# YAIconvalley/distributed-pipeline

Measured on AMD Instinct MI355X. Metric: train steps/sec (whole node), DiffuSeq-base seq128 DDP at 1/2/4/8 MI355X, higher is better.
Workload: dtype bf16

## Files before the change

### distributed_pipeline_amd/csrc/vocab_sweep.h

```cpp
#pragma once
#include <type_traits>

#include "common.h"
#include "mfma.h"

namespace dpa {

template <int E, int NT>
struct WTile {
  static constexpr int CH = E / 8;
  static constexpr int ROWB = E * 2;
  static constexpr int PER = 64 * CH / NT;
  uint4 r[PER];

  __device__ __forceinline__ void load(const bf16_t* __restrict__ W, int v0, int V, int tid) {
#pragma unroll
    for (int i = 0; i < PER; ++i) {
      const int c = tid + i * NT;
      const int row = c / CH, ch = c % CH;
      const int v = v0 + row;
      if (v < V)
        r[i] = *reinterpret_cast<const uint4*>(W + (int64_t)v * E + ch * 8);
      else
        r[i] = make_uint4(0, 0, 0, 0);
    }
  }
  __device__ __forceinline__ void store(char* lds, int tid) const {
#pragma unroll
    for (int i = 0; i < PER; ++i) {
      const int c = tid + i * NT;
      const int row = c / CH, ch = c % CH;
      *reinterpret_cast<uint4*>(lds + swz<ROWB>(row, ch)) = r[i];
    }
  }
};

template <int E>
__device__ __forceinline__ bf16x8 token_frag(const bf16_t* __restrict__ x, int t, bool tok_ok, int s, int h) {
  bf16x8 f;
  if (tok_ok) f = ld_frag(x + (int64_t)t * E + 16 * s + 8 * h);
  else for (int j = 0; j < 8; ++j) f[j] = 0;
  return f;
}

template <class F>
__device__ __forceinline__ void stage_offsets(float* bt, int v0, int vend, int tid, F offset) {
  if (tid < 64) {
    const int v = v0 + tid;
    bt[tid] = (v < vend) ? offset(v) : -INFINITY;
  }
}

struct SweepBlock {
  int split, tblk, nsplit;
};
__device__ __forceinline__ SweepBlock sweep_block(int xsplit) {
  SweepBlock b;
  b.split = xsplit > 1 ? (int)(blockIdx.x % xsplit) : (int)blockIdx.y;
  b.tblk = xsplit > 1 ? (int)(blockIdx.x / xsplit) : (int)blockIdx.x;
  b.nsplit = xsplit > 1 ? xsplit : (int)gridDim.y;
  return b;
}

inline int pick_splits(int blocks, int chunks, int target_wgs) {
  int s = (target_wgs + blocks - 1) / blocks;
  if (s < 1) s = 1;
  if (s > chunks) s = chunks;
  return s;
}

enum class XcdRound { none, if_split, always };

struct SweepPlan {
  int tb;
  int Sx;
  int vps;
};

inline SweepPlan sweep_plan(int N, int V, int target_wgs, XcdRound xcd) {
  const int tb = (N + 127) / 128, vchunks = (V + 63) / 64;
  int S = pick_splits(tb, vchunks, target_wgs);
  if (vchunks >= 8 && (xcd == XcdRound::always || (xcd == XcdRound::if_split && S > 1))) S = (S + 7) / 8 * 8;
  const int vps = ((vchunks + S - 1) / S) * 64;
  return {tb, (V + vps - 1) / vps, vps};
}

template <class F>
inline void for_head_width(int E, F f) {
  if (E == 128) f(std::integral_constant<int, 128>{});
  else f(std::integral_constant<int, 256>{});
}

}
```

### distributed_pipeline_amd/csrc/xent.hip

```cpp
#include <cstdlib>

#include <type_traits>

#include "common.h"
#include "launchers.h"
#include "mfma.h"
#include "vocab_sweep.h"

namespace dpa {

static constexpr float LN2 = 0.6931471805599453f;

struct BiasOffset {
  const bf16_t* bias;
  __device__ __forceinline__ float operator()(int v) const { return bias ? bf2f(bias[v]) : 0.f; }
};

__device__ __forceinline__ float sel16(const f32x16& a, int i) {
  float v = 0.f;
#pragma unroll
  for (int k = 0; k < 16; ++k) v = (k == i) ? a[k] : v;
  return v;
}

template <int E>
__global__ void __launch_bounds__(256) lxent_fwd_kernel(
    const bf16_t* __restrict__ x, const bf16_t* __restrict__ W, const bf16_t* __restrict__ bias,
    const int64_t* __restrict__ target, int N, int V, int v_per_split, float* __restrict__ loss,
    float* __restrict__ lse_out, float* __restrict__ part_m, float* __restrict__ part_s,
    float* __restrict__ tgt_logit, int xsplit) {
  constexpr int KS = E / 16, ROWB = E * 2;
  __shared__ __attribute__((aligned(16))) char smem[64 * ROWB + 64 * 4];
  char* wt = smem;
  float* bt = reinterpret_cast<float*>(smem + 64 * ROWB);

  const auto [split, tblk, nsplit] = sweep_block(xsplit);
  const int tid = threadIdx.x, lane = tid & 63, w = tid >> 6, h = lane >> 5;
  const int t = tblk * 128 + w * 32 + (lane & 31);
  const bool tok_ok = t < N;
  bf16x8 xf[KS];
#pragma unroll
  for (int s = 0; s < KS; ++s) xf[s] = token_frag<E>(x, t, tok_ok, s, h);
  const int64_t tg = tok_ok ? target[t] : -1;

  const int vbeg = split * v_per_split;
  const int vend = min(V, vbeg + v_per_split);
  if (!__syncthreads_or(tg >= 0 && tg < V)) {
    if (h == 0 && tok_ok) {
      if (nsplit == 1) {
        loss[t] = 0.f;
        lse_out[t] = 0.f;
      } else {
        part_m[(int64_t)split * N + t] = 0.f;
        part_s[(int64_t)split * N + t] = 1.f;
      }
    }
    return;
  }
  float m = -1e30f, ssum = 0.f, tl = -INFINITY;

  WTile<E, 256> stage;
  if (vbeg < vend) stage.load(W, vbeg, V, tid);
  for (int v0 = vbeg; v0 < vend; v0 += 64) {
    stage.store(wt, tid);
    stage_offsets(bt, v0, vend, tid, BiasOffset{bias});
    __syncthreads();
    if (v0 + 64 < vend) stage.load(W, v0 + 64, V, tid);

    f32x16 acc[2];
#pragma unroll
    for (int vt = 0; vt < 2; ++vt) {
#pragma unroll
      for (int g = 0; g < 4; ++g) {
        const f32x4 bv = *reinterpret_cast<const f32x4*>(bt + vt * 32 + 8 * g + 4 * h);
#pragma unroll
        for (int r = 0; r < 4; ++r) acc[vt][4 * g + r] = bv[r];
      }
#pragma unroll
      for (int s = 0; s < KS; ++s)
        acc[vt] = mfma32(lds_frag<ROWB>(wt, vt * 32 + (lane & 31), 2 * s + h), xf[s], acc[vt]);
    }
    float tmax = -INFINITY;
#pragma unroll
    for (int vt = 0; vt < 2; ++vt)
#pragma unroll
      for (int i = 0; i < 16; i += 2) tmax = fmaxf(tmax, fmaxf(acc[vt][i], acc[vt][i + 1]));
    const float mn = fmaxf(m, tmax * LOG2E);
    float add = 0.f;
#pragma unroll
    for (int vt = 0; vt < 2; ++vt)
#pragma unroll
      for (int i = 0; i < 16; ++i) add += fexp2(fmaf(acc[vt][i], LOG2E, -mn));
    ssum = ssum * fexp2(m - mn) + add;
    m = mn;
    const int64_t r = tg - v0;
    if (r >= 0 && r < 64 && v0 + r < vend) {
      const int rr = (int)r & 31, vt = (int)r >> 5;
      if (((rr >> 2) & 1) == h) {
        const int i = (rr & 3) + 4 * (rr >> 3);
        tl = vt ? sel16(acc[1], i) : sel16(acc[0], i);
      }
    }
    __syncthreads();
  }
  const float m2 = __shfl_xor(m, 32, 64), s2 = __shfl_xor(ssum, 32, 64);
  const float tl2 = __shfl_xor(tl, 32, 64);
  const float M = fmaxf(m, m2);
  const float S = ssum * fexp2(m - M) + s2 * fexp2(m2 - M);
  tl = fmaxf(tl, tl2);
  if (h == 0 && tok_ok) {
    if (nsplit == 1) {
      const bool valid = tg >= 0 && tg < V;
      const float lse = (M + log2f(S)) * LN2;
      loss[t] = valid ? lse - tl : 0.f;
      lse_out[t] = lse;
    } else {
      part_m[(int64_t)split * N + t] = M;
      part_s[(int64_t)split * N + t] = S;
      if (tl > -INFINITY) tgt_logit[t] = tl;
    }
  }
}

__global__ void __launch_bounds__(256) lxent_combine_kernel(
    const float* __restrict__ part_m, const float* __restrict__ part_s,
    const float* __restrict__ tgt_logit, const int64_t* __restrict__ target, int N, int V, int S,
    float* __restrict__ loss, float* __restrict__ lse_out) {
  const int t = blockIdx.x * blockDim.x + threadIdx.x;
  if (t >= N) return;
  float M = -1e30f;
  for (int s = 0; s < S; ++s) M = fmaxf(M, part_m[(int64_t)s * N + t]);
  float sum = 0.f;
  for (int s = 0; s < S; ++s) sum += part_s[(int64_t)s * N + t] * fexp2(part_m[(int64_t)s * N + t] - M);
  const float lse = (M + log2f(sum)) * LN2;
  const int64_t tg = target[t];
  const bool valid = tg >= 0 && tg < V;
  loss[t] = valid ? lse - tgt_logit[t] : 0.f;
  lse_out[t] = lse;
}

template <int E>
__global__ void __launch_bounds__(256) lxent_dx_kernel(
    const bf16_t* __restrict__ x, const bf16_t* __restrict__ W, const bf16_t* __restrict__ bias,
    const int64_t* __restrict__ target, const float* __restrict__ lse, const float* __restrict__ dloss,
    int N, int V, int v_per_split, bf16_t* __restrict__ dx, float* __restrict__ dx_acc) {
  constexpr int KS = E / 16, ROWB = E * 2, KT = E / 32;
  __shared__ __attribute__((aligned(16))) char smem[64 * ROWB + 64 * 4];
  char* wt = smem;
  float* bt = reinterpret_cast<float*>(smem + 64 * ROWB);

  const int tid = threadIdx.x, lane = tid & 63, w = tid >> 6, h = lane >> 5;
  const int t = blockIdx.x * 128 + w * 32 + (lane & 31);
  const bool tok_ok = t < N;
  bf16x8 xf[KS];
#pragma unroll
  for (int s = 0; s < KS; ++s) xf[s] = token_frag<E>(x, t, tok_ok, s, h);
  const int64_t tg = tok_ok ? target[t] : -1;
  const bool valid = tok_ok && tg >= 0 && tg < V;
  const float g = valid ? dloss[t] : 0.f;
  const float lse2 = tok_ok ? lse[t] * LOG2E : 0.f;

  const int vbeg = blockIdx.y * v_per_split;
  const int vend = min(V, vbeg + v_per_split);
  f32x16 dacc[KT];
#pragma unroll
  for (int k = 0; k < KT; ++k) dacc[k] = zero16();

  WTile<E, 256> stage;
  if (vbeg < vend) stage.load(W, vbeg, V, tid);
  for (int v0 = vbeg; v0 < vend; v0 += 64) {
    stage.store(wt, tid);
    stage_offsets(bt, v0, vend, tid, BiasOffset{bias});
    __syncthreads();
    if (v0 + 64 < vend) stage.load(W, v0 + 64, V, tid);

#pragma unroll
    for (int vt = 0; vt < 2; ++vt) {
      f32x16 acc;
#pragma unroll
      for (int g4 = 0; g4 < 4; ++g4) {
        const f32x4 bv = *reinterpret_cast<const f32x4*>(bt + vt * 32 + 8 * g4 + 4 * h);
#pragma unroll
        for (int r = 0; r < 4; ++r) acc[4 * g4 + r] = bv[r];
      }
#pragma unroll
      for (int s = 0; s < KS; ++s)
        acc = mfma32(lds_frag<ROWB>(wt, vt * 32 + (lane & 31), 2 * s + h), xf[s], acc);
#pragma unroll
      for (int i = 0; i < 16; ++i) acc[i] = g * fexp2(fmaf(acc[i], LOG2E, -lse2));
      const int64_t rt = tg - (v0 + vt * 32);
      if (rt >= 0 && rt < 32 && tg < vend && ((rt >> 2) & 1) == h) {
        const int it = ((int)rt & 3) + 4 * ((int)rt >> 3);
#pragma unroll
        for (int i = 0; i < 16; ++i) acc[i] -= (i == it) ? g : 0.f;
      }
#pragma unroll
      for (int s = 0; s < 2; ++s) {
        const bf16x8 af = acc_to_frag(acc, s);
#pragma unroll
        for (int kt = 0; kt < KT; ++kt)
          dacc[kt] = mfma32(af, lds_tr_frag<ROWB>(wt, vt * 32 + 16 * s, kt * 32, lane), dacc[kt]);
      }
    }
    __syncthreads();
  }
  const int tb = blockIdx.x * 128 + w * 32;
#pragma unroll
  for (int kt = 0; kt < KT; ++kt) {
#pragma unroll
    for (int i = 0; i < 16; ++i) {
      const int tt = tb + acc_row(i, h);
      if (tt < N) {
        const int64_t o = (int64_t)tt * E + kt * 32 + (lane & 31);
        if (dx_acc) atomicAdd(dx_acc + o, dacc[kt][i]);
        else dx[o] = f2bf(dacc[kt][i]);
      }
    }
  }
}

template <int E>
__global__ void __launch_bounds__(256, E == 128 ? 2 : 1) lxent_fwd_dx_kernel(
    const bf16_t* __restrict__ x, const bf16_t* __restrict__ W, const bf16_t* __restrict__ bias,
    const int64_t* __restrict__ target, int N, int V, float* __restrict__ loss,
    float* __restrict__ lse_out, float* __restrict__ dxu, int vps, float* __restrict__ part) {
  constexpr int KS = E / 16, ROWB = E * 2, KT = E / 32;
  __shared__ __attribute__((aligned(16))) char smem[64 * ROWB + 64 * 4];
  const int v_lo = part ? (int)blockIdx.y * vps : 0;
  const int v_hi = part ? min(V, v_lo + vps) : V;
  char* wt = smem;
  float* bt = reinterpret_cast<float*>(smem + 64 * ROWB);

  const int tid = threadIdx.x, lane = tid & 63, w = tid >> 6, h = lane >> 5;
  const int t = blockIdx.x * 128 + w * 32 + (lane & 31);
  const bool tok_ok = t < N;
  bf16x8 xf[KS];
#pragma unroll
  for (int s = 0; s < KS; ++s) xf[s] = token_frag<E>(x, t, tok_ok, s, h);
  const int64_t tg = tok_ok ? target[t] : -1;
  f32x16 dacc[KT];
#pragma unroll
  for (int k = 0; k < KT; ++k) dacc[k] = zero16();
  float m = -1e30f, l = 0.f, tl = -INFINITY;

  WTile<E, 256> stage;
  stage.load(W, v_lo, V, tid);
  for (int v0 = v_lo; v0 < v_hi; v0 += 64) {
    stage.store(wt, tid);
    stage_offsets(bt, v0, v_hi, tid, BiasOffset{bias});
    __syncthreads();
    if (v0 + 64 < v_hi) stage.load(W, v0 + 64, V, tid);

#pragma unroll
    for (int vt = 0; vt < 2; ++vt) {
      f32x16 acc;
#pragma unroll
      for (int g = 0; g < 4; ++g) {
        const f32x4 bv = *reinterpret_cast<const f32x4*>(bt + vt * 32 + 8 * g + 4 * h);
#pragma unroll
        for (int r = 0; r < 4; ++r) acc[4 * g + r] = bv[r];
      }
#pragma unroll
      for (int s = 0; s < KS; ++s)
        acc = mfma32(lds_frag<ROWB>(wt, vt * 32 + (lane & 31), 2 * s + h), xf[s], acc);
      const int64_t r = tg - (v0 + vt * 32);
      if (r >= 0 && r < 32 && ((((int)r >> 2) & 1) == h)) tl = sel16(acc, ((int)r & 3) + 4 * ((int)r >> 3));
      float tmax = -INFINITY;
#pragma unroll
      for (int i = 0; i < 16; ++i) tmax = fmaxf(tmax, acc[i]);
      tmax = fmaxf(tmax, __shfl_xor(tmax, 32, 64)) * LOG2E;
      if (__any(tmax > m + 8.f)) {
        const float mn = fmaxf(m, tmax);
        const float alpha = fexp2(m - mn);
        m = mn;
        l *= alpha;
#pragma unroll
        for (int i = 0; i < 16; ++i) {
          const float f = __shfl(alpha, acc_row(i, h), 64);
#pragma unroll
          for (int kt = 0; kt < KT; ++kt) dacc[kt][i] *= f;
        }
      }
#pragma unroll
      for (int i = 0; i < 16; ++i) {
        const float pr = fexp2(fmaf(acc[i], LOG2E, -m));
        l += pr;
        acc[i] = pr;
      }
#pragma unroll
      for (int s = 0; s < 2; ++s) {
        const bf16x8 af = acc_to_frag(acc, s);
#pragma unroll
        for (int kt = 0; kt < KT; ++kt)
          dacc[kt] = mfma32(af, lds_tr_frag<ROWB>(wt, vt * 32 + 16 * s, kt * 32, lane), dacc[kt]);
      }
    }
    __syncthreads();
  }
  l += __shfl_xor(l, 32, 64);
  tl = fmaxf(tl, __shfl_xor(tl, 32, 64));
  if (part) {
    const int S = gridDim.y, sp = blockIdx.y;
    float* pm = part;
    float* pl = pm + (int64_t)S * N;
    float* pt = pl + (int64_t)S * N;
    float* pu = pt + (int64_t)S * N;
    if (h == 0 && tok_ok) {
      pm[(int64_t)sp * N + t] = m;
      pl[(int64_t)sp * N + t] = l;
      pt[(int64_t)sp * N + t] = tl;
    }
    const int tb0 = blockIdx.x * 128 + w * 32;
#pragma unroll
    for (int i = 0; i < 16; ++i) {
      const int tt = tb0 + acc_row(i, h);
      if (tt < N) {
#pragma unroll
        for (int kt = 0; kt < KT; ++kt) pu[((int64_t)sp * N + tt) * E + kt * 32 + (lane & 31)] = dacc[kt][i];
      }
    }
    return;
  }
  const bool valid = tok_ok && tg >= 0 && tg < V;
  const float lse = (m + log2f(l)) * LN2;
  if (h == 0 && tok_ok) {
    loss[t] = valid ? lse - tl : 0.f;
    lse_out[t] = lse;
  }
  const float inv_l = valid ? 1.f / l : 0.f;
  const int tb = blockIdx.x * 128 + w * 32;
#pragma unroll
  for (int i = 0; i < 16; ++i) {
    const int src = acc_row(i, h);
    const float f = __shfl(inv_l, src, 64);
    const int64_t tgi = __shfl(tg, src, 64);
    const int tt = tb + src;
    if (tt < N) {
#pragma unroll
      for (int kt = 0; kt < KT; ++kt) {
        const int k = kt * 32 + (lane & 31);
        float vv = 0.f;
        if (f != 0.f) vv = dacc[kt][i] * f - bf2f(W[tgi * E + k]);
        dxu[(int64_t)tt * E + k] = vv;
      }
    }
  }
}

template <int E>
__global__ void __launch_bounds__(256) lxent_fwd_dx_combine_kernel(
    const float* __restrict__ part, int S, const bf16_t* __restrict__ W, const int64_t* __restrict__ target,
    int N, int V, float* __restrict__ loss, float* __restrict__ lse_out, float* __restrict__ dxu) {
  const int64_t idx = (int64_t)blockIdx.x * blockDim.x + threadIdx.x;
  if (idx >= (int64_t)N * E) return;
  const int t = (int)(idx / E), k = (int)(idx % E);
  const float* pm = part;
  const float* pl = pm + (int64_t)S * N;
  const float* pt = pl + (int64_t)S * N;
  const float* pu = pt + (int64_t)S * N;
  float M = -1e30f, tl = -INFINITY;
  for (int s = 0; s < S; ++s) {
    M = fmaxf(M, pm[(int64_t)s * N + t]);
    tl = fmaxf(tl, pt[(int64_t)s * N + t]);
  }
  float L = 0.f, u = 0.f;
  for (int s = 0; s < S; ++s) {
    const float f = fexp2(pm[(int64_t)s * N + t] - M);
    L += pl[(int64_t)s * N + t] * f;
    u += pu[((int64_t)s * N + t) * E + k] * f;
  }
  const int64_t tg = target[t];
  const bool valid = tg >= 0 && tg < V;
  const float lse = (M + log2f(L)) * LN2;
  if (k == 0) {
    loss[t] = valid ? lse - tl : 0.f;
    lse_out[t] = lse;
  }
  dxu[(int64_t)t * E + k] = valid ? u / L - bf2f(W[tg * E + k]) : 0.f;
}

template <int E, bool ONEHOT = true>
__global__ void __launch_bounds__(512) lxent_dw_kernel(
    const bf16_t* __restrict__ x, const bf16_t* __restrict__ W, const bf16_t* __restrict__ bias,
    const int64_t* __restrict__ target, const float* __restrict__ lse, const float* __restrict__ dloss,
    int N, int V, int t_per_split, float* __restrict__ dW, float* __restrict__ db, float* __restrict__ ws) {
  constexpr int KS = E / 16, ROWB = E * 2, KT = E / 32, CH = E / 8;
  __shared__ __attribute__((aligned(16))) char smem[64 * ROWB + 3 * 64 * 4];
  char* xt = smem;
  float* s_lse = reinterpret_cast<float*>(smem + 64 * ROWB);
  float* s_g = s_lse + 64;
  int* s_tg = reinterpret_cast<int*>(s_g + 64);

  const int tid = threadIdx.x, lane = tid & 63, w = tid >> 6, h = lane >> 5;
  if (w < 4) __builtin_amdgcn_s_setprio(1);
  const int vw = blockIdx.x * 256 + w * 32;
  const int v = vw + (lane & 31);
  const bool v_ok = v < V;
  bf16x8 wf[KS];
#pragma unroll
  for (int s = 0; s < KS; ++s) {
    if (v_ok) wf[s] = ld_frag(W + (int64_t)v * E + 16 * s + 8 * h);
    else for (int j = 0; j < 8; ++j) wf[s][j] = 0;
  }
  const float bv = v_ok ? (bias ? bf2f(bias[v]) : 0.f) : -INFINITY;

  f32x16 dacc[KT];
#pragma unroll
  for (int k = 0; k < KT; ++k) dacc[k] = zero16();
  float dbs = 0.f;

  const int tbeg = blockIdx.y * t_per_split;
  const int tend = min(N, tbeg + t_per_split);
  constexpr int PER = 64 * CH / 512;
  uint4 xr[PER];
  float r_lse = 0.f, r_g = 0.f;
  int r_tg = -1;
  auto load_tile = [&](int t0) {
#pragma unroll
    for (int i = 0; i < PER; ++i) {
      const int c = tid + i * 512;
      const int t = t0 + c / CH;
      xr[i] = t < tend ? *reinterpret_cast<const uint4*>(x + (int64_t)t * E + (c % CH) * 8)
                       : make_uint4(0, 0, 0, 0);
    }
    if (tid < 64) {
      const int t = t0 + tid;
      const bool ok = t < tend;
      const int64_t tg = ok ? target[t] : -1;
      const bool valid = ok && tg >= 0 && tg < V;
      r_lse = ok ? lse[t] * LOG2E : 0.f;
      r_g = valid ? dloss[t] : 0.f;
      r_tg = valid ? (int)tg : -1;
    }
  };
  if (tbeg < tend) load_tile(tbeg);
  for (int t0 = tbeg; t0 < tend; t0 += 64) {
#pragma unroll
    for (int i = 0; i < PER; ++i) {
      const int c = tid + i * 512;
      *reinterpret_cast<uint4*>(xt + swz<ROWB, true>(c / CH, c % CH)) = xr[i];
    }
    if (tid < 64) {
      s_lse[tid] = r_lse;
      s_g[tid] = r_g;
      s_tg[tid] = r_tg;
    }
    __syncthreads();
    if (t0 + 64 < tend) load_tile(t0 + 64);
#pragma unroll
    for (int tt = 0; tt < 2; ++tt) {
      f32x16 acc;
#pragma unroll
      for (int i = 0; i < 16; ++i) acc[i] = bv;
#pragma unroll
      for (int s = 0; s < KS; ++s)
        acc = mfma32(lds_frag<ROWB, true>(xt, tt * 32 + (lane & 31), 2 * s + h), wf[s], acc);
      auto softmax_grad = [&](auto oh) {
        constexpr bool OH = decltype(oh)::value;
#pragma unroll
        for (int g4 = 0; g4 < 4; ++g4) {
          const int rb = tt * 32 + 8 * g4 + 4 * h;
          const f32x4 l4 = *reinterpret_cast<const f32x4*>(s_lse + rb);
          const f32x4 g4v = *reinterpret_cast<const f32x4*>(s_g + rb);
          int tgs[4] = {-1, -1, -1, -1};
          if constexpr (OH) {
            const int4 t4 = *reinterpret_cast<const int4*>(s_tg + rb);
            tgs[0] = t4.x; tgs[1] = t4.y; tgs[2] = t4.z; tgs[3] = t4.w;
          }
#pragma unroll
          for (int r = 0; r < 4; ++r) {
            const int i = 4 * g4 + r;
            const float gp = g4v[r] * fexp2(fmaf(acc[i], LOG2E, -l4[r]));
            const float d = (OH && tgs[r] == v) ? gp - g4v[r] : gp;
            acc[i] = d;
            dbs += d;
          }
        }
      };
      bool hit = false;
      if constexpr (ONEHOT) {
        const int tgl = s_tg[tt * 32 + (lane & 31)];
        hit = __any(tgl >= vw && tgl < vw + 32);
      }
      if (hit) softmax_grad(std::true_type{});
      else softmax_grad(std::false_type{});
#pragma unroll
      for (int s = 0; s < 2; ++s) {
        const bf16x8 af = acc_to_frag(acc, s);
#pragma unroll
        for (int kt = 0; kt < KT; ++kt)
          dacc[kt] = mfma32(af, lds_tr_frag<ROWB, true>(xt, tt * 32 + 16 * s, kt * 32, lane), dacc[kt]);
      }
    }
    __syncthreads();
  }
  dbs += __shfl_xor(dbs, 32, 64);
  float* const pw = ws ? ws + (int64_t)blockIdx.y * V * (E + 1) : nullptr;
  if (h == 0 && v_ok && db) {
    if (pw) pw[(int64_t)V * E + v] = dbs;
    else db[v] += dbs;
  }
#pragma unroll
  for (int kt = 0; kt < KT; ++kt) {
#pragma unroll
    for (int i = 0; i < 16; ++i) {
      const int vv = vw + acc_row(i, h);
      if (vv < V) {
        const int64_t o = (int64_t)vv * E + kt * 32 + (lane & 31);
        if (pw) pw[o] = dacc[kt][i];
        else dW[o] += dacc[kt][i];
      }
    }
  }
}

__global__ void __launch_bounds__(256) xent_split_reduce_kernel(const float* __restrict__ ws, int64_t stride,
                                                                int splits, int64_t n, float* __restrict__ dst) {
  const int64_t i = (int64_t)blockIdx.x * blockDim.x + threadIdx.x;
  if (i >= n) return;
  float a = dst[i];
  for (int sp = 0; sp < splits; ++sp) a += ws[(int64_t)sp * stride + i];
  dst[i] = a;
}

__global__ void __launch_bounds__(256) f32_to_bf16_kernel(const float* __restrict__ a,
                                                         bf16_t* __restrict__ b, int64_t n) {
  const int64_t i = ((int64_t)blockIdx.x * blockDim.x + threadIdx.x) * 4;
  if (i + 3 < n) {
    f32x4 v = *reinterpret_cast<const f32x4*>(a + i);
    uint2 p;
    p.x = pack_bf2(v[0], v[1]);
    p.y = pack_bf2(v[2], v[3]);
    *reinterpret_cast<uint2*>(b + i) = p;
  } else {
    for (int64_t k = i; k < n; ++k) b[k] = f2bf(a[k]);
  }
}

static SweepPlan fwd_plan(int N, int V) { return sweep_plan(N, V, 1024, XcdRound::always); }

int64_t lxent_workspace_floats(int N, int V) { return (2 * (int64_t)fwd_plan(N, V).Sx + 1) * N + 64; }

void launch_lxent_fwd(const uint16_t* x, const uint16_t* W, const uint16_t* b, const int64_t* tgt,
                      int N, int V, int E, float* loss, float* lse, float* ws, hipStream_t s) {
  const SweepPlan p = fwd_plan(N, V);
  float* pm = ws;
  float* ps = ws + (int64_t)p.Sx * N;
  float* tl = ws + 2 * (int64_t)p.Sx * N;
  const bool per_xcd = p.Sx == 8;
  const dim3 grid = per_xcd ? dim3(p.tb * 8) : dim3(p.tb, p.Sx);
  for_head_width(E, [&](auto e) {
    hipLaunchKernelGGL(lxent_fwd_kernel<e()>, grid, dim3(256), 0, s, x, W, b, tgt, N, V, p.vps, loss, lse, pm,
                       ps, tl, per_xcd ? 8 : 0);
  });
  if (p.Sx > 1)
    hipLaunchKernelGGL(lxent_combine_kernel, dim3((N + 255) / 256), dim3(256), 0, s, pm, ps, tl,
                       tgt, N, V, p.Sx, loss, lse);
}

static SweepPlan fwd_dx_plan(int N, int V) { return sweep_plan(N, V, 768, XcdRound::none); }

int64_t lxent_fwd_dx_workspace_floats(int N, int V, int E) {
  const int S = fwd_dx_plan(N, V).Sx;
  return S > 1 ? (int64_t)S * N * (3 + E) : 0;
}

void launch_lxent_fwd_dx(const uint16_t* x, const uint16_t* W, const uint16_t* b, const int64_t* tgt,
                         int N, int V, int E, float* loss, float* lse, float* dxu, hipStream_t s, float* ws) {
  const SweepPlan p = fwd_dx_plan(N, V);
  for_head_width(E, [&](auto e) {
    if (p.Sx > 1 && ws != nullptr) {
      hipLaunchKernelGGL(lxent_fwd_dx_kernel<e()>, dim3(p.tb, p.Sx), dim3(256), 0, s, x, W, b, tgt, N, V, loss,
                         lse, dxu, p.vps, ws);
      const int64_t n = (int64_t)N * E;
      hipLaunchKernelGGL(lxent_fwd_dx_combine_kernel<e()>, dim3((unsigned)((n + 255) / 256)), dim3(256), 0, s, ws,
                         p.Sx, W, tgt, N, V, loss, lse, dxu);
    } else {
      hipLaunchKernelGGL(lxent_fwd_dx_kernel<e()>, dim3(p.tb), dim3(256), 0, s, x, W, b, tgt, N, V, loss, lse,
                         dxu, V, nullptr);
    }
  });
}

bool lxent_dx_needs_acc(int N) { return (N + 127) / 128 < 512; }

void launch_lxent_dx(const uint16_t* x, const uint16_t* W, const uint16_t* b, const int64_t* tgt,
                     const float* lse, const float* dloss, int N, int V, int E, uint16_t* dx,
                     float* dx_acc, hipStream_t s) {
  const SweepPlan p = sweep_plan(N, V, dx_acc ? 1024 : 0, XcdRound::none);
  for_head_width(E, [&](auto e) {
    hipLaunchKernelGGL(lxent_dx_kernel<e()>, dim3(p.tb, p.Sx), dim3(256), 0, s, x, W, b, tgt, lse, dloss, N, V,
                       p.vps, dx, p.Sx > 1 ? dx_acc : nullptr);
  });
  if (p.Sx > 1) {
    const int64_t n = (int64_t)N * E;
    hipLaunchKernelGGL(f32_to_bf16_kernel, dim3((unsigned)((n / 4 + 255) / 256 + 1)), dim3(256), 0,
                       s, dx_acc, dx, n);
  }
}

static void lxent_dw_plan(int N, int V, int& vb, int& tps, int& TSx) {
  vb = (V + 255) / 256;
  const int tchunks = (N + 63) / 64;
  const int TS = pick_splits(vb, tchunks, 960);
  tps = ((tchunks + TS - 1) / TS) * 64;
  TSx = (N + tps - 1) / tps;
}

int64_t lxent_dw_ws_floats(int N, int V, int E) {
  int vb, tps, TSx;
  lxent_dw_plan(N, V, vb, tps, TSx);
  return TSx > 1 ? (int64_t)TSx * V * (E + 1) : 0;
}

void launch_lxent_dw(const uint16_t* x, const uint16_t* W, const uint16_t* b, const int64_t* tgt,
                     const float* lse, const float* dloss, int N, int V, int E, float* dW, float* db,
                     hipStream_t s, bool onehot, float* ws) {
  int vb, tps, TSx;
  lxent_dw_plan(N, V, vb, tps, TSx);
  float* wsp = TSx > 1 ? ws : nullptr;
#define DPA_LXDW(EE, OH)                                                                                \
  hipLaunchKernelGGL((lxent_dw_kernel<EE, OH>), dim3(vb, TSx), dim3(512), 0, s, (const bf16_t*)x,        \
                     (const bf16_t*)W, (const bf16_t*)b, tgt, lse, dloss, N, V, tps, dW, db, wsp)
  if (E == 128) {
    if (onehot) DPA_LXDW(128, true); else DPA_LXDW(128, false);
  } else {
    if (onehot) DPA_LXDW(256, true); else DPA_LXDW(256, false);
  }
#undef DPA_LXDW
  if (wsp) {
    const int64_t stride = (int64_t)V * (E + 1), nw = (int64_t)V * E;
    hipLaunchKernelGGL(xent_split_reduce_kernel, dim3((unsigned)((nw + 255) / 256)), dim3(256), 0, s,
                       (const float*)wsp, stride, TSx, nw, dW);
    if (db)
      hipLaunchKernelGGL(xent_split_reduce_kernel, dim3((unsigned)((V + 255) / 256)), dim3(256), 0, s,
                         (const float*)(wsp + nw), stride, TSx, (int64_t)V, db);
  }
}

}
```

Before: 6.195.

## Stream vocab/token tiles through a 3-stage LDS ring with direct buffer-to-LDS loads

New measurement: 6.245 (median of 6 runs). About the same (+0.8%).

```diff
diff --git a/distributed_pipeline_amd/csrc/vocab_sweep.h b/distributed_pipeline_amd/csrc/vocab_sweep.h
--- a/distributed_pipeline_amd/csrc/vocab_sweep.h
+++ b/distributed_pipeline_amd/csrc/vocab_sweep.h
@@ -1,5 +1,6 @@
 #pragma once
 #include <type_traits>
+#include <utility>
 
 #include "common.h"
 #include "mfma.h"
@@ -35,6 +36,205 @@
   }
 };
 
+typedef __attribute__((address_space(3))) void lds_void;
+
+struct RingSched {
+  int R;
+  constexpr int slot(int tile) const { return ((tile % R) + R) % R; }
+  constexpr int tiles_in_flight_at_wait() const { return R - 2; }
+  constexpr int published(int tile) const { return tile; }
+  constexpr int first_read(int tile) const { return tile; }
+  constexpr int last_read(int tile) const { return tile + 1; }
+  constexpr int fill_after(int tile) const { return tile <= R - 2 ? -0x7fffffff : tile - R + 1; }
+  constexpr int barriers(int T) const { return T > 0 ? T : 0; }
+};
+constexpr bool ring_schedule_ok(RingSched s, int T) {
+  if (s.R < 3 || s.tiles_in_flight_at_wait() != 1) return false;
+  if (s.barriers(T) != T) return false;
+  for (int j = 0; j < T + s.R - 1; ++j) {
+    if (j < T && s.first_read(j) < s.published(j)) return false;
+    if (j < T && s.published(j) < s.fill_after(j)) return false;
+    if (j >= s.R && s.slot(j) != s.slot(j - s.R)) return false;
+    if (j >= s.R && s.fill_after(j) < s.last_read(j - s.R)) return false;
+  }
+  return true;
+}
+constexpr bool ring_schedule_ok_all(RingSched s) {
+  const int trips[8] = {0, 1, 2, s.R - 1, s.R, s.R + 1, s.R + 2, 477};
+  for (int k = 0; k < 8; ++k)
+    if (!ring_schedule_ok(s, trips[k])) return false;
+  return true;
+}
+
+template <int N>
+__device__ __forceinline__ void ring_wait_vm() { asm volatile("s_waitcnt vmcnt(%0)" ::"i"(N) : "memory"); }
+__device__ __forceinline__ void ring_barrier() { asm volatile("s_waitcnt lgkmcnt(0)\n\ts_barrier" ::: "memory"); }
+
+template <int OFF>
+__device__ __forceinline__ bf16x8 ring_rd128(uint32_t a) {
+  bf16x8 f;
+  asm volatile("ds_read_b128 %0, %1 offset:%2" : "=v"(f) : "v"(a), "i"(OFF));
+  return f;
+}
+template <int OFF>
+__device__ __forceinline__ f32x4 ring_rd_f4(uint32_t a) {
+  f32x4 f;
+  asm volatile("ds_read_b128 %0, %1 offset:%2" : "=v"(f) : "v"(a), "i"(OFF));
+  return f;
+}
+typedef __attribute__((ext_vector_type(4))) int i32x4;
+template <int OFF>
+__device__ __forceinline__ i32x4 ring_rd_i4(uint32_t a) {
+  i32x4 f;
+  asm volatile("ds_read_b128 %0, %1 offset:%2" : "=v"(f) : "v"(a), "i"(OFF));
+  return f;
+}
+template <int OFF>
+__device__ __forceinline__ int ring_rd_i1(uint32_t a) {
+  int f;
+  asm volatile("ds_read_b32 %0, %1 offset:%2" : "=v"(f) : "v"(a), "i"(OFF));
+  return f;
+}
+template <int OFF>
+__device__ __forceinline__ bf16x4 ring_rdtr(uint32_t a) {
+  bf16x4 f;
+  asm volatile("ds_read_b64_tr_b16 %0, %1 offset:%2" : "=v"(f) : "v"(a), "i"(OFF));
+  return f;
+}
+__device__ __forceinline__ void ring_wr_b32(uint32_t a, uint32_t v) {
+  asm volatile("ds_write_b32 %0, %1" ::"v"(a), "v"(v) : "memory");
+}
+template <int N, class T>
+__device__ __forceinline__ void ring_lgkm(T& f) { asm volatile("s_waitcnt lgkmcnt(%1)" : "+v"(f) : "i"(N)); }
+template <int N, class T>
+__device__ __forceinline__ void ring_lgkm(T& f, T& g) {
+  asm volatile("s_waitcnt lgkmcnt(%2)" : "+v"(f), "+v"(g) : "i"(N));
+}
+
+__device__ __forceinline__ uint32_t ring_ld_u16(const void* p) {
+  uint32_t v;
+  asm volatile("global_load_ushort %0, %1, off" : "=v"(v) : "v"(p));
+  return v;
+}
+__device__ __forceinline__ uint32_t ring_ld_b32(const void* p) {
+  uint32_t v;
+  asm volatile("global_load_dword %0, %1, off" : "=v"(v) : "v"(p));
+  return v;
+}
+__device__ __forceinline__ int64_t ring_ld_b64(const void* p) {
+  int64_t v;
+  asm volatile("global_load_dwordx2 %0, %1, off" : "=v"(v) : "v"(p));
+  return v;
+}
+template <int N, class T>
+__device__ __forceinline__ void ring_wait_vm_on(T& a) {
+  asm volatile("s_waitcnt vmcnt(%1)" : "+v"(a) : "i"(N) : "memory");
+}
+
+template <int E, int NW, int R, int SIDE, bool LEG>
+struct TileRing {
+  static constexpr int ROWB = E * 2, CH = E / 8, TILE = 64 * ROWB;
+  static constexpr int PER = TILE / 1024 / NW;
+  static constexpr int TAIL = SIDE * 256;
+  static constexpr int BYTES = R * (TILE + TAIL);
+  static constexpr int KS = E / 16, KT = E / 32;
+  static_assert(ROWB % 256 == 0 && ROWB <= 1024 && PER >= 1 && PER * NW * 1024 == TILE, "tile shape");
+
+  char* smem;
+  uint32_t base;
+  uint32_t off[PER];
+  uint32_t rdA[KS];
+  uint32_t rdT[KT][2];
+  int wv;
+
+  __device__ __forceinline__ void init(char* smem_, int tid) {
+    smem = smem_;
+    base = (uint32_t)reinterpret_cast<uintptr_t>((const __attribute__((address_space(3))) char*)smem_);
+    const int lane = tid & 63, h = lane >> 5;
+    wv = __builtin_amdgcn_readfirstlane(tid >> 6);
+#pragma unroll
+    for (int j = 0; j < PER; ++j) {
+      const int row = (wv * PER + j) * (64 / CH) + lane / CH, phys = lane % CH;
+      off[j] = (uint32_t)(row * ROWB + ((phys ^ swz_x256<LEG>(row)) << 4));
+    }
+#pragma unroll
+    for (int s = 0; s < KS; ++s) rdA[s] = (uint32_t)swz<ROWB, LEG>(lane & 31, 2 * s + h);
+    const int g = lane >> 4, li = lane & 15, q = li >> 2, p = li & 3;
+#pragma unroll
+    for (int kt = 0; kt < KT; ++kt) {
+      const int col = kt * 32 + 16 * (g & 1) + 4 * p, ra = 4 * h + q;
+      rdT[kt][0] = (uint32_t)(swz<ROWB, LEG>(ra, col >> 3) + (col & 7) * 2);
+      rdT[kt][1] = (uint32_t)(swz<ROWB, LEG>(ra + 8, col >> 3) + (col & 7) * 2);
+    }
+  }
+  __device__ __forceinline__ uint32_t tile_addr(int slot) const { return base + (uint32_t)(slot * TILE); }
+  __device__ __forceinline__ uint32_t tail_addr(int slot) const { return base + (uint32_t)(R * TILE + slot * TAIL); }
+
+  __device__ __forceinline__ void fill(int slot, const bf16_t* __restrict__ src, int row0, int rows) const {
+    const int n = __builtin_amdgcn_readfirstlane(min(max(rows - row0, 0), 64));
+    const bf16_t* p = src + (n > 0 ? (int64_t)row0 * E : 0);
+    const auto rs = __builtin_amdgcn_make_buffer_rsrc(const_cast<bf16_t*>(p), (short)0, n * ROWB, 0x00020000);
+#pragma unroll
+    for (int j = 0; j < PER; ++j)
+      __builtin_amdgcn_raw_ptr_buffer_load_lds(rs, (lds_void*)(smem + slot * TILE + (wv * PER + j) * 1024), 16,
+                                               off[j], 0, 0, 0);
+  }
+};
+
+template <class Ring, int VT, int J>
+__device__ __forceinline__ void ring_logits_step(f32x16& acc, bf16x8 (&f)[4], const Ring& r, uint32_t ta,
+                                                 const bf16x8 (&b)[Ring::KS]) {
+  constexpr int KS = Ring::KS, N = KS - 1 - J < 3 ? KS - 1 - J : 3;
+  ring_lgkm<N>(f[J % 4]);
+  acc = mfma32(f[J % 4], b[J], acc);
+  if constexpr (J + 4 < KS) f[J % 4] = ring_rd128<VT * 32 * Ring::ROWB>(ta + r.rdA[J + 4]);
+}
+template <class Ring, int VT, int... J>
+__device__ __forceinline__ void ring_logits_steps(f32x16& acc, bf16x8 (&f)[4], const Ring& r, uint32_t ta,
+                                                  const bf16x8 (&b)[Ring::KS], std::integer_sequence<int, J...>) {
+  (ring_logits_step<Ring, VT, J>(acc, f, r, ta, b), ...);
+}
+template <class Ring, int VT, class Init>
+__device__ __forceinline__ void ring_logits(f32x16& acc, const Ring& r, uint32_t ta,
+                                            const bf16x8 (&b)[Ring::KS], Init init) {
+  bf16x8 f[4];
+#pragma unroll
+  for (int j = 0; j < 4; ++j) f[j] = ring_rd128<VT * 32 * Ring::ROWB>(ta + r.rdA[j]);
+  init(acc);
+  ring_logits_steps<Ring, VT>(acc, f, r, ta, b, std::make_integer_sequence<int, Ring::KS>{});
+}
+
+struct TrChunk {
+  bf16x4 a[4], b[4];
+};
+template <class Ring, int VT, int C>
+__device__ __forceinline__ void ring_tr_issue(TrChunk& c, const Ring& r, uint32_t ta) {
+  constexpr int S = C / (Ring::KT / 4), KT0 = 4 * (C % (Ring::KT / 4)), OFF = (VT * 32 + 16 * S) * Ring::ROWB;
+#pragma unroll
+  for (int k = 0; k < 4; ++k) {
+    c.a[k] = ring_rdtr<OFF>(ta + r.rdT[KT0 + k][0]);
+    c.b[k] = ring_rdtr<OFF>(ta + r.rdT[KT0 + k][1]);
+  }
+}
+template <class Ring, int VT, int C = 0>
+__device__ __forceinline__ void ring_acc_mfma(f32x16 (&dacc)[Ring::KT], const f32x16& acc, const Ring& r,
+                                              uint32_t ta, TrChunk& cur) {
+  constexpr int NCH = Ring::KT / 2, S = C / (Ring::KT / 4), KT0 = 4 * (C % (Ring::KT / 4));
+  constexpr int P = C + 1 < NCH ? 8 : 0;
+  const bf16x8 af = acc_to_frag(acc, S);
+  TrChunk nxt;
+  ring_lgkm<6>(cur.a[0], cur.b[0]);
+  if constexpr (C + 1 < NCH) ring_tr_issue<Ring, VT, C + 1>(nxt, r, ta);
+  dacc[KT0] = mfma32(af, cat44(cur.a[0], cur.b[0]), dacc[KT0]);
+  ring_lgkm<P + 4>(cur.a[1], cur.b[1]);
+  dacc[KT0 + 1] = mfma32(af, cat44(cur.a[1], cur.b[1]), dacc[KT0 + 1]);
+  ring_lgkm<P + 2>(cur.a[2], cur.b[2]);
+  dacc[KT0 + 2] = mfma32(af, cat44(cur.a[2], cur.b[2]), dacc[KT0 + 2]);
+  ring_lgkm<P>(cur.a[3], cur.b[3]);
+  dacc[KT0 + 3] = mfma32(af, cat44(cur.a[3], cur.b[3]), dacc[KT0 + 3]);
+  if constexpr (C + 1 < NCH) ring_acc_mfma<Ring, VT, C + 1>(dacc, acc, r, ta, nxt);
+}
+
 template <int E>
 __device__ __forceinline__ bf16x8 token_frag(const bf16_t* __restrict__ x, int t, bool tok_ok, int s, int h) {
   bf16x8 f;
diff --git a/distributed_pipeline_amd/csrc/xent.hip b/distributed_pipeline_amd/csrc/xent.hip
--- a/distributed_pipeline_amd/csrc/xent.hip
+++ b/distributed_pipeline_amd/csrc/xent.hip
@@ -15,6 +15,14 @@
   const bf16_t* bias;
   __device__ __forceinline__ float operator()(int v) const { return bias ? bf2f(bias[v]) : 0.f; }
 };
+
+constexpr int FWD_DX_STAGES = 3, DW_STAGES = 3;
+template <int E> using FwdDxRing = TileRing<E, 4, FWD_DX_STAGES, 1, false>;
+template <int E> using DwRing = TileRing<E, 8, DW_STAGES, 3, true>;
+static_assert(ring_schedule_ok_all(RingSched{FWD_DX_STAGES}), "lxent_fwd_dx ring schedule");
+static_assert(ring_schedule_ok_all(RingSched{DW_STAGES}), "lxent_dw ring schedule");
+static_assert(2 * FwdDxRing<128>::BYTES <= 160 * 1024 && FwdDxRing<256>::BYTES <= 160 * 1024 &&
+              DwRing<256>::BYTES <= 160 * 1024, "the rings of a CU's resident blocks fit its LDS");
 
 __device__ __forceinline__ float sel16(const f32x16& a, int i) {
   float v = 0.f;
@@ -224,14 +232,16 @@
     const bf16_t* __restrict__ x, const bf16_t* __restrict__ W, const bf16_t* __restrict__ bias,
     const int64_t* __restrict__ target, int N, int V, float* __restrict__ loss,
     float* __restrict__ lse_out, float* __restrict__ dxu, int vps, float* __restrict__ part) {
-  constexpr int KS = E / 16, ROWB = E * 2, KT = E / 32;
-  __shared__ __attribute__((aligned(16))) char smem[64 * ROWB + 64 * 4];
+  constexpr int KS = E / 16, KT = E / 32;
+  using Ring = FwdDxRing<E>;
+  constexpr int R = FWD_DX_STAGES, PER = Ring::PER;
+  __shared__ __attribute__((aligned(1024))) char smem[Ring::BYTES];
   const int v_lo = part ? (int)blockIdx.y * vps : 0;
   const int v_hi = part ? min(V, v_lo + vps) : V;
-  char* wt = smem;
-  float* bt = reinterpret_cast<float*>(smem + 64 * ROWB);
 
   const int tid = threadIdx.x, lane = tid & 63, w = tid >> 6, h = lane >> 5;
+  Ring ring;
+  ring.init(smem, tid);
   const int t = blockIdx.x * 128 + w * 32 + (lane & 31);
   const bool tok_ok = t < N;
   bf16x8 xf[KS];
@@ -243,26 +253,64 @@
   for (int k = 0; k < KT; ++k) dacc[k] = zero16();
   float m = -1e30f, l = 0.f, tl = -INFINITY;
 
-  WTile<E, 256> stage;
-  stage.load(W, v_lo, V, tid);
-  for (int v0 = v_lo; v0 < v_hi; v0 += 64) {
-    stage.store(wt, tid);
-    stage_offsets(bt, v0, v_hi, tid, BiasOffset{bias});
-    __syncthreads();
-    if (v0 + 64 < v_hi) stage.load(W, v0 + 64, V, tid);
-
-#pragma unroll
-    for (int vt = 0; vt < 2; ++vt) {
+  const bool side_wave = ring.wv == 0;
+  auto side_load = [&](int j) -> uint32_t {
+    return bias ? ring_ld_u16(bias + min(v_lo + 64 * j + tid, v_hi - 1)) : 0u;
+  };
+  auto side_store = [&](int j, int slot, uint32_t raw) {
+    const float o = v_lo + 64 * j + tid < v_hi ? (bias ? bf2f((bf16_t)raw) : 0.f) : -INFINITY;
+    ring_wr_b32(ring.tail_addr(slot) + 4 * tid, __float_as_uint(o));
+  };
+  uint32_t snext = 0;
+  {
+    uint32_t sraw[R];
+    if (side_wave) {
+#pragma unroll
+      for (int j = 0; j < R; ++j) sraw[j] = side_load(j);
+    }
+#pragma unroll
+    for (int j = 0; j < R - 1; ++j) ring.fill(j, W, v_lo + 64 * j, v_hi);
+    if (side_wave) {
+#pragma unroll
+      for (int j = 0; j < R; ++j) ring_wait_vm_on<(R - 1) * PER>(sraw[j]);
+#pragma unroll
+      for (int j = 0; j < R - 1; ++j) side_store(j, j, sraw[j]);
+      snext = sraw[R - 1];
+    }
+  }
+  const int tiles = (v_hi - v_lo + 63) / 64;
+  int slot = 0;
+  for (int it = 0; it < tiles; ++it) {
+    const int v0 = v_lo + 64 * it;
+    ring_wait_vm_on<PER>(snext);
+    ring_barrier();
+    {
+      const int fslot = slot == 0 ? R - 1 : slot - 1;
+      if (side_wave) {
+        side_store(it + R - 1, fslot, snext);
+        snext = side_load(it + R);
+      }
+      ring.fill(fslot, W, v0 + 64 * (R - 1), v_hi);
+    }
+    const uint32_t ta = ring.tile_addr(slot), sa = ring.tail_addr(slot) + 16 * h;
+    slot = slot == R - 1 ? 0 : slot + 1;
+
+    auto subtile = [&](auto vtc) {
+      constexpr int vt = decltype(vtc)::value;
       f32x16 acc;
-#pragma unroll
-      for (int g = 0; g < 4; ++g) {
-        const f32x4 bv = *reinterpret_cast<const f32x4*>(bt + vt * 32 + 8 * g + 4 * h);
-#pragma unroll
-        for (int r = 0; r < 4; ++r) acc[4 * g + r] = bv[r];
-      }
-#pragma unroll
-      for (int s = 0; s < KS; ++s)
-        acc = mfma32(lds_frag<ROWB>(wt, vt * 32 + (lane & 31), 2 * s + h), xf[s], acc);
+      f32x4 bv[4];
+#pragma unroll
+      for (int g = 0; g < 4; ++g) bv[g] = ring_rd_f4<vt * 128>(sa + 32 * g);
+      ring_logits<Ring, vt>(acc, ring, ta, xf, [&](f32x16& a) {
+        ring_lgkm<4>(bv[0], bv[1]);
+        ring_lgkm<4>(bv[2], bv[3]);
+#pragma unroll
+        for (int g = 0; g < 4; ++g)
+#pragma unroll
+          for (int r = 0; r < 4; ++r) a[4 * g + r] = bv[g][r];
+      });
+      TrChunk tr;
+      ring_tr_issue<Ring, vt, 0>(tr, ring, ta);
       const int64_t r = tg - (v0 + vt * 32);
       if (r >= 0 && r < 32 && ((((int)r >> 2) & 1) == h)) tl = sel16(acc, ((int)r & 3) + 4 * ((int)r >> 3));
       float tmax = -INFINITY;
@@ -287,16 +335,12 @@
         l += pr;
         acc[i] = pr;
       }
-#pragma unroll
-      for (int s = 0; s < 2; ++s) {
-        const bf16x8 af = acc_to_frag(acc, s);
-#pragma unroll
-        for (int kt = 0; kt < KT; ++kt)
-          dacc[kt] = mfma32(af, lds_tr_frag<ROWB>(wt, vt * 32 + 16 * s, kt * 32, lane), dacc[kt]);
-      }
-    }
-    __syncthreads();
-  }
+      ring_acc_mfma<Ring, vt>(dacc, acc, ring, ta, tr);
+    };
+    subtile(std::integral_constant<int, 0>{});
+    subtile(std::integral_constant<int, 1>{});
+  }
+  ring_wait_vm<0>();
   l += __shfl_xor(l, 32, 64);
   tl = fmaxf(tl, __shfl_xor(tl, 32, 64));
   if (part) {
@@ -384,15 +428,14 @@
     const bf16_t* __restrict__ x, const bf16_t* __restrict__ W, const bf16_t* __restrict__ bias,
     const int64_t* __restrict__ target, const float* __restrict__ lse, const float* __restrict__ dloss,
     int N, int V, int t_per_split, float* __restrict__ dW, float* __restrict__ db, float* __restrict__ ws) {
-  constexpr int KS = E / 16, ROWB = E * 2, KT = E / 32, CH = E / 8;
-  __shared__ __attribute__((aligned(16))) char smem[64 * ROWB + 3 * 64 * 4];
-  char* xt = smem;
-  float* s_lse = reinterpret_cast<float*>(smem + 64 * ROWB);
-  float* s_g = s_lse + 64;
-  int* s_tg = reinterpret_cast<int*>(s_g + 64);
+  constexpr int KS = E / 16, KT = E / 32;
+  using Ring = DwRing<E>;
+  constexpr int R = DW_STAGES, PER = Ring::PER;
+  __shared__ __attribute__((aligned(1024))) char smem[Ring::BYTES];
 
   const int tid = threadIdx.x, lane = tid & 63, w = tid >> 6, h = lane >> 5;
-  if (w < 4) __builtin_amdgcn_s_setprio(1);
+  Ring ring;
+  ring.init(smem, tid);
   const int vw = blockIdx.x * 256 + w * 32;
   const int v = vw + (lane & 31);
   const bool v_ok = v < V;
@@ -411,67 +454,98 @@
 
   const int tbeg = blockIdx.y * t_per_split;
   const int tend = min(N, tbeg + t_per_split);
-  constexpr int PER = 64 * CH / 512;
-  uint4 xr[PER];
-  float r_lse = 0.f, r_g = 0.f;
-  int r_tg = -1;
-  auto load_tile = [&](int t0) {
-#pragma unroll
-    for (int i = 0; i < PER; ++i) {
-      const int c = tid + i * 512;
-      const int t = t0 + c / CH;
-      xr[i] = t < tend ? *reinterpret_cast<const uint4*>(x + (int64_t)t * E + (c % CH) * 8)
-                       : make_uint4(0, 0, 0, 0);
-    }
-    if (tid < 64) {
-      const int t = t0 + tid;
-      const bool ok = t < tend;
-      const int64_t tg = ok ? target[t] : -1;
-      const bool valid = ok && tg >= 0 && tg < V;
-      r_lse = ok ? lse[t] * LOG2E : 0.f;
-      r_g = valid ? dloss[t] : 0.f;
-      r_tg = valid ? (int)tg : -1;
-    }
+  const int tiles = (tend - tbeg + 63) / 64;
+  const bool side_wave = ring.wv == 0;
+  struct Side {
+    uint32_t l, g;
+    int64_t t;
   };
-  if (tbeg < tend) load_tile(tbeg);
-  for (int t0 = tbeg; t0 < tend; t0 += 64) {
-#pragma unroll
-    for (int i = 0; i < PER; ++i) {
-      const int c = tid + i * 512;
-      *reinterpret_cast<uint4*>(xt + swz<ROWB, true>(c / CH, c % CH)) = xr[i];
-    }
-    if (tid < 64) {
-      s_lse[tid] = r_lse;
-      s_g[tid] = r_g;
-      s_tg[tid] = r_tg;
-    }
-    __syncthreads();
-    if (t0 + 64 < tend) load_tile(t0 + 64);
-#pragma unroll
-    for (int tt = 0; tt < 2; ++tt) {
+  auto side_load = [&](int j) {
+    const int t = max(min(tbeg + 64 * j + tid, tend - 1), 0);
+    return Side{ring_ld_b32(lse + t), ring_ld_b32(dloss + t), ring_ld_b64(target + t)};
+  };
+  auto side_store = [&](int j, int slot, const Side& sd) {
+    const bool ok = tbeg + 64 * j + tid < tend;
+    const bool valid = ok && sd.t >= 0 && sd.t < V;
+    const uint32_t a = ring.tail_addr(slot) + 4 * tid;
+    ring_wr_b32(a, __float_as_uint(ok ? __uint_as_float(sd.l) * LOG2E : 0.f));
+    ring_wr_b32(a + 256, valid ? sd.g : 0u);
+    ring_wr_b32(a + 512, (uint32_t)(valid ? (int)sd.t : -1));
+  };
+  Side snext{0u, 0u, 0};
+  if (tiles > 0) {
+    Side sraw[R];
+    if (side_wave) {
+#pragma unroll
+      for (int j = 0; j < R; ++j) sraw[j] = side_load(j);
+    }
+#pragma unroll
+    for (int j = 0; j < R - 1; ++j) ring.fill(j, x, tbeg + 64 * j, tend);
+    if (side_wave) {
+#pragma unroll
+      for (int j = 0; j < R; ++j) {
+        ring_wait_vm_on<(R - 1) * PER>(sraw[j].l);
+        ring_wait_vm_on<(R - 1) * PER>(sraw[j].g);
+        ring_wait_vm_on<(R - 1) * PER>(sraw[j].t);
+      }
+#pragma unroll
+      for (int j = 0; j < R - 1; ++j) side_store(j, j, sraw[j]);
+      snext = sraw[R - 1];
+    }
+  }
+  int slot = 0;
+  for (int it = 0; it < tiles; ++it) {
+    ring_wait_vm_on<PER>(snext.l);
+    ring_wait_vm_on<PER>(snext.g);
+    ring_wait_vm_on<PER>(snext.t);
+    const uint32_t ta = ring.tile_addr(slot), sa = ring.tail_addr(slot);
+    ring_barrier();
+    {
+      const int fslot = slot == 0 ? R - 1 : slot - 1;
+      if (side_wave) {
+        side_store(it + R - 1, fslot, snext);
+        snext = side_load(it + R);
+      }
+      ring.fill(fslot, x, tbeg + 64 * (it + R - 1), tend);
+    }
+    slot = slot == R - 1 ? 0 : slot + 1;
+    auto set_bias = [&](f32x16& a) {
+#pragma unroll
+      for (int i = 0; i < 16; ++i) a[i] = bv;
+    };
+    auto subtile = [&](auto ttc) {
+      constexpr int tt = decltype(ttc)::value;
       f32x16 acc;
-#pragma unroll
-      for (int i = 0; i < 16; ++i) acc[i] = bv;
-#pragma unroll
-      for (int s = 0; s < KS; ++s)
-        acc = mfma32(lds_frag<ROWB, true>(xt, tt * 32 + (lane & 31), 2 * s + h), wf[s], acc);
+      ring_logits<Ring, tt>(acc, ring, ta, wf, set_bias);
+      int tgl = 0;
+      if constexpr (ONEHOT) tgl = ring_rd_i1<512 + tt * 128>(sa + 4 * (lane & 31));
+      f32x4 l4[4], g4v[4];
+#pragma unroll
+      for (int g4 = 0; g4 < 4; ++g4) {
+        l4[g4] = ring_rd_f4<tt * 128>(sa + 32 * g4 + 16 * h);
+        g4v[g4] = ring_rd_f4<256 + tt * 128>(sa + 32 * g4 + 16 * h);
+      }
+      TrChunk tr;
       auto softmax_grad = [&](auto oh) {
         constexpr bool OH = decltype(oh)::value;
 #pragma unroll
         for (int g4 = 0; g4 < 4; ++g4) {
-          const int rb = tt * 32 + 8 * g4 + 4 * h;
-          const f32x4 l4 = *reinterpret_cast<const f32x4*>(s_lse + rb);
-          const f32x4 g4v = *reinterpret_cast<const f32x4*>(s_g + rb);
+          if (g4 == 0) ring_lgkm<6>(l4[0], g4v[0]);
+          else if (g4 == 1) ring_lgkm<12>(l4[1], g4v[1]);
+          else if (g4 == 2) ring_lgkm<10>(l4[2], g4v[2]);
+          else ring_lgkm<8>(l4[3], g4v[3]);
+          if (g4 == 0) ring_tr_issue<Ring, tt, 0>(tr, ring, ta);
           int tgs[4] = {-1, -1, -1, -1};
           if constexpr (OH) {
-            const int4 t4 = *reinterpret_cast<const int4*>(s_tg + rb);
-            tgs[0] = t4.x; tgs[1] = t4.y; tgs[2] = t4.z; tgs[3] = t4.w;
+            i32x4 t4 = ring_rd_i4<512 + tt * 128>(sa + 32 * g4 + 16 * h);
+            ring_lgkm<0>(t4);
+            tgs[0] = t4[0]; tgs[1] = t4[1]; tgs[2] = t4[2]; tgs[3] = t4[3];
           }
 #pragma unroll
           for (int r = 0; r < 4; ++r) {
             const int i = 4 * g4 + r;
-            const float gp = g4v[r] * fexp2(fmaf(acc[i], LOG2E, -l4[r]));
-            const float d = (OH && tgs[r] == v) ? gp - g4v[r] : gp;
+            const float gp = g4v[g4][r] * fexp2(fmaf(acc[i], LOG2E, -l4[g4][r]));
+            const float d = (OH && tgs[r] == v) ? gp - g4v[g4][r] : gp;
             acc[i] = d;
             dbs += d;
           }
@@ -479,21 +553,17 @@
       };
       bool hit = false;
       if constexpr (ONEHOT) {
-        const int tgl = s_tg[tt * 32 + (lane & 31)];
+        ring_lgkm<8>(tgl);
         hit = __any(tgl >= vw && tgl < vw + 32);
       }
       if (hit) softmax_grad(std::true_type{});
       else softmax_grad(std::false_type{});
-#pragma unroll
-      for (int s = 0; s < 2; ++s) {
-        const bf16x8 af = acc_to_frag(acc, s);
-#pragma unroll
-        for (int kt = 0; kt < KT; ++kt)
-          dacc[kt] = mfma32(af, lds_tr_frag<ROWB, true>(xt, tt * 32 + 16 * s, kt * 32, lane), dacc[kt]);
-      }
-    }
-    __syncthreads();
-  }
+      ring_acc_mfma<Ring, tt>(dacc, acc, ring, ta, tr);
+    };
+    subtile(std::integral_constant<int, 0>{});
+    subtile(std::integral_constant<int, 1>{});
+  }
+  ring_wait_vm<0>();
   dbs += __shfl_xor(dbs, 32, 64);
   float* const pw = ws ? ws + (int64_t)blockIdx.y * V * (E + 1) : nullptr;
   if (h == 0 && v_ok && db) {
@@ -513,6 +583,16 @@
     }
   }
 }
+
+#define DPA_LXDW_INST(EE, OH)                                                                           \
+  template __global__ void lxent_dw_kernel<EE, OH>(const bf16_t*, const bf16_t*, const bf16_t*, const int64_t*, \
+                                                   const float*, const float*, int, int, int, float*, float*,   \
+                                                   float*)
+DPA_LXDW_INST(128, true);
+DPA_LXDW_INST(128, false);
+DPA_LXDW_INST(256, true);
+DPA_LXDW_INST(256, false);
+#undef DPA_LXDW_INST
 
 __global__ void __launch_bounds__(256) xent_split_reduce_kernel(const float* __restrict__ ws, int64_t stride,
                                                                 int splits, int64_t n, float* __restrict__ dst) {
```
